# xuhao1/TaichiSLAM

Measured on AMD Instinct MI355X. Metric: depth-frames/s integrated (640x480->512^3 TSDF), higher is better.
Workload: dtype f16 storage / f32 + int64 fixed-point arithmetic; 1 GPU; BASELINE configs[1]: single 640x480 u16 depth stream (sphere room r=3 m, 1 deg/frame) -> DenseTSDF 512^3 / 2 cm, recast_step 2, max_ray 5 m; one stream+submap per GPU

## Files before the change

taichislam_amd/csrc/tsl_common.hpp:

```cpp
#pragma once
#include <cstring>
#include <string.h>
#include <hip/hip_runtime.h>
#include <stdint.h>
#include <string>
#include <vector>
#include "../../include/taichislam_hip.h"

#define TSL_BRK   16
#define TSL_BRK3  4096
#define TSL_EMPTY  (-1)
#define TSL_LOCKED (-2)
#define TSL_FULL   (-3)

namespace tsl {

void set_error(const std::string& s);
#define TSL_HIP(expr) do { hipError_t _e = (expr); if (_e != hipSuccess) { \
    tsl::set_error(std::string(#expr) + ": " + hipGetErrorString(_e)); return TSL_ERR_HIP; } } while (0)
#define TSL_REQUIRE(cond, msg) do { if (!(cond)) { tsl::set_error(msg); return TSL_ERR_ARG; } } while (0)

typedef uint16_t h16;
__device__ __forceinline__ h16 f2h(float x) { _Float16 v = (_Float16)x; return __builtin_bit_cast(h16, v); }
__device__ __forceinline__ float h2f(h16 b) { return (float)__builtin_bit_cast(_Float16, b); }
__device__ __forceinline__ h16 hadd(h16 a, h16 b) { return f2h(h2f(a) + h2f(b)); }
__device__ __forceinline__ h16 hsub(h16 a, h16 b) { return f2h(h2f(a) - h2f(b)); }
__device__ __forceinline__ h16 hmul(h16 a, h16 b) { return f2h(h2f(a) * h2f(b)); }
__device__ __forceinline__ h16 hdiv(h16 a, h16 b) { return f2h(h2f(a) / h2f(b)); }
__device__ __forceinline__ float sqrt_rn(float x) { return sqrtf(x); }
__device__ __forceinline__ float sqrt_rn_norm(float x)
{
    const float y = __builtin_amdgcn_sqrtf(x);
    const float yd = __uint_as_float(__float_as_uint(y) - 1u), yu = __uint_as_float(__float_as_uint(y) + 1u);
    const float ed = __builtin_fmaf(-yd, y, x), eu = __builtin_fmaf(-yu, y, x);
    float r = (ed <= 0.0f) ? yd : y;
    r = (eu > 0.0f) ? yu : r;
    return r;
}
__device__ __forceinline__ h16 hsqrt(h16 a) { return f2h(sqrt_rn(h2f(a))); }

__device__ __forceinline__ float rnd_f(float x)
{
    float r = truncf(x);
    float d = fabsf(x - r);
    if (d >= 0.5f) r += copysignf(1.0f, x);
    return r;
}
__device__ __forceinline__ int rnd_i(float x) { return (int)(x + copysignf(0.49999997f, x)); }
__device__ __forceinline__ int rnd_i_ref(float x) { return (int)rnd_f(x); }
__device__ __forceinline__ int sgn_f(float v) { return (0.0f < v) - (v < 0.0f); }

__device__ __forceinline__ float div_vs(float x, float vs, float rvs, int fast)
{
    if (fast) { const float q0 = x * rvs; const float r = __builtin_fmaf(-q0, vs, x); return __builtin_fmaf(r, rvs, q0); }
    return x / vs;
}

#define TSL_FIX_SCALE 16777216.0f
#define TSL_FIX_INV   (1.0 / 16777216.0)
#define TSL_W_CLAMP   65536.0f
#define TSL_WMAX      1000.0f
__device__ __forceinline__ long long to_fix(float v)
{
    const float q = rintf(v * TSL_FIX_SCALE);
    if (fabsf(q) < 2147483648.0f) return (long long)(int)q;
    return __float2ll_rn(q);
}
__device__ __forceinline__ long long to_fix_wave(float v)
{
    const float q = rintf(v * TSL_FIX_SCALE);
    if (__builtin_expect(__any(!(fabsf(q) < 2147483648.0f)), 0)) return __float2ll_rn(q);
    return (long long)(int)q;
}
__device__ __forceinline__ float from_fix(long long q) { return (float)((double)q * TSL_FIX_INV); }

__device__ __forceinline__ int lane_id() { return __builtin_amdgcn_mbcnt_hi(~0u, __builtin_amdgcn_mbcnt_lo(~0u, 0u)); }
__device__ __forceinline__ int popc64(unsigned long long m) { return __popcll(m); }
__device__ __forceinline__ int rank_below(unsigned long long m)
{ return __builtin_amdgcn_mbcnt_hi((unsigned)(m >> 32), __builtin_amdgcn_mbcnt_lo((unsigned)m, 0u)); }

__device__ __forceinline__ void atomic_add_i64(int64_t* ctr, long long v)
{ __hip_atomic_fetch_add(reinterpret_cast<long long*>(ctr), v, __ATOMIC_RELAXED, __HIP_MEMORY_SCOPE_AGENT); }
__device__ __forceinline__ void wave_count_add(int64_t* ctr, bool pred)
{
    unsigned long long m = __ballot(pred);
    if (m && lane_id() == (int)__builtin_ctzll(m)) atomic_add_i64(ctr, (long long)popc64(m));
}
__device__ __forceinline__ void block_count_add(int64_t* ctr, bool pred)
{
    __shared__ int s_cnt;
    if (threadIdx.x == 0) s_cnt = 0;
    __syncthreads();
    unsigned long long m = __ballot(pred);
    if (m && lane_id() == (int)__builtin_ctzll(m)) atomicAdd(&s_cnt, popc64(m));
    __syncthreads();
    if (threadIdx.x == 0 && s_cnt) atomic_add_i64(ctr, (long long)s_cnt);
    __syncthreads();
}
__device__ __forceinline__ long long wave_sum_ll(long long v)
{
    for (int d = 32; d > 0; d >>= 1) v += __shfl_xor(v, d);
    return v;
}
__device__ __forceinline__ int wave_reserve(int* ctr, bool pred)
{
    unsigned long long m = __ballot(pred);
    if (!m) return -1;
    int leader = (int)__builtin_ctzll(m);
    int base = 0;
    if (lane_id() == leader) base = __hip_atomic_fetch_add(ctr, popc64(m), __ATOMIC_RELAXED, __HIP_MEMORY_SCOPE_AGENT);
    base = __shfl(base, leader);
    return pred ? base + rank_below(m) : -1;
}

__device__ __forceinline__ int block_reserve_n(int* ctr, int n)
{
    __shared__ int s_w[4];
    __shared__ int s_b;
    const int lane = lane_id(), wid = threadIdx.x >> 6;
    int inc = n;
    for (int d = 1; d < 64; d <<= 1) { const int o = __shfl_up(inc, d); if (lane >= d) inc += o; }
    if (lane == 63) s_w[wid] = inc;
    __syncthreads();
    if (threadIdx.x == 0) {
        const int tot = s_w[0] + s_w[1] + s_w[2] + s_w[3];
        s_b = tot ? __hip_atomic_fetch_add(ctr, tot, __ATOMIC_RELAXED, __HIP_MEMORY_SCOPE_AGENT) : 0;
    }
    __syncthreads();
    int off = s_b + inc - n;
    for (int w = 0; w < wid; ++w) off += s_w[w];
    __syncthreads();
    return off;
}

__device__ __forceinline__ int block_reserve(int* ctr, bool pred)
{
    __shared__ int s_w[4];
    __shared__ int s_b;
    const unsigned long long m = __ballot(pred);
    const int wid = threadIdx.x >> 6;
    if (lane_id() == 0) s_w[wid] = popc64(m);
    __syncthreads();
    if (threadIdx.x == 0) {
        const int tot = s_w[0] + s_w[1] + s_w[2] + s_w[3];
        s_b = tot ? __hip_atomic_fetch_add(ctr, tot, __ATOMIC_RELAXED, __HIP_MEMORY_SCOPE_AGENT) : 0;
    }
    __syncthreads();
    int off = s_b + rank_below(m);
    for (int w = 0; w < wid; ++w) off += s_w[w];
    __syncthreads();
    return pred ? off : -1;
}

__device__ __forceinline__ int claim_index_1(int* entry, int* counter, int cap)
{
    int v = __hip_atomic_load(entry, __ATOMIC_RELAXED, __HIP_MEMORY_SCOPE_AGENT);
    while (v == TSL_EMPTY || v == TSL_LOCKED) {
        if (v == TSL_EMPTY) {
            int old = atomicCAS(entry, TSL_EMPTY, TSL_LOCKED);
            if (old == TSL_EMPTY) {
                int idx = __hip_atomic_load(counter, __ATOMIC_RELAXED, __HIP_MEMORY_SCOPE_AGENT);
                if (idx < cap) idx = __hip_atomic_fetch_add(counter, 1, __ATOMIC_RELAXED, __HIP_MEMORY_SCOPE_AGENT);
                __hip_atomic_store(entry, idx >= cap ? TSL_EMPTY : idx, __ATOMIC_RELAXED, __HIP_MEMORY_SCOPE_AGENT);
                return idx >= cap ? TSL_FULL : idx;
            }
            v = old;
        } else {
            __builtin_amdgcn_s_sleep(2);
            v = __hip_atomic_load(entry, __ATOMIC_RELAXED, __HIP_MEMORY_SCOPE_AGENT);
        }
    }
    return v;
}
__device__ __forceinline__ int claim_index(int* entry, int* counter, int cap)
{
    int v = __hip_atomic_load(entry, __ATOMIC_RELAXED, __HIP_MEMORY_SCOPE_AGENT);
    unsigned long long todo = __ballot(v == TSL_EMPTY || v == TSL_LOCKED);
    while (todo) {
        const int leader = (int)__builtin_ctzll(todo);
        const unsigned long long lead = __shfl((unsigned long long)entry, leader);
        int r = 0;
        if (lane_id() == leader) r = claim_index_1(entry, counter, cap);
        r = __shfl(r, leader);
        const bool mine = ((unsigned long long)entry == lead);
        if (mine) v = r;
        todo &= ~__ballot(mine);
    }
    return v;
}

struct MapDev {
    int N, Nz, nbx, nbz, nb3, nsub;
    int hN, hNz;
    int max_bricks;
    int* table;
    uint32_t* tw;
    int8_t* obs;
    int8_t* occ;
    uint16_t* col;
    int* owner;
    uint8_t* touch;
    int* pool_top;
    int* err;
};

__device__ __forceinline__ bool in_volume(const MapDev& M, int i, int j, int k)
{
    return i >= -M.hN && i < M.N - M.hN && j >= -M.hN && j < M.N - M.hN && k >= -M.hNz && k < M.Nz - M.hNz;
}
__device__ __forceinline__ int brick_of(const MapDev& M, int i, int j, int k, int* local)
{
    int ui = i + M.hN, uj = j + M.hN, uk = k + M.hNz;
    *local = ((ui & 15) << 8) | ((uj & 15) << 4) | (uk & 15);
    return ((ui >> 4) * M.nbx + (uj >> 4)) * M.nbz + (uk >> 4);
}
__device__ __forceinline__ int pool_lookup(const MapDev& M, int s, int b)
{ return __hip_atomic_load(M.table + (size_t)s * M.nb3 + b, __ATOMIC_RELAXED, __HIP_MEMORY_SCOPE_AGENT); }
__device__ __forceinline__ int pool_lookup_ro(const MapDev& M, int s, int b) { return M.table[(size_t)s * M.nb3 + b]; }
template <bool COOP = true>
__device__ __forceinline__ int pool_claim(const MapDev& M, int s, int b)
{
    int* e = M.table + (size_t)s * M.nb3 + b;
    int v = __hip_atomic_load(e, __ATOMIC_RELAXED, __HIP_MEMORY_SCOPE_AGENT);
    if (v >= 0) return v;
    v = COOP ? claim_index(e, M.pool_top, M.max_bricks) : claim_index_1(e, M.pool_top, M.max_bricks);
    if (v >= 0) M.owner[v] = s * M.nb3 + b;
    else atomicOr(M.err, 1);
    return v;
}

__device__ __forceinline__ void fuse_write_voxel(const MapDev& G, size_t v, long long qn, long long qd, int c)
{
    const int occ_sum = (int)(int16_t)(c & 0xffff);
    const float num = from_fix(qn), den = from_fix(qd);
    G.tw[v] = (uint32_t)f2h(num / den) | ((uint32_t)f2h(den) << 16);
    G.obs[v] = 1;
    G.occ[v] = (int8_t)occ_sum;
}


}
```

taichislam_amd/csrc/tsl_integrate.hip:

```cpp
#include "tsl_tsdf.hpp"
#include <hip/hip_ext.h>

namespace tsl {

#ifdef TSL_TIMING
#define TSL_T0() const int _wv = (blockIdx.x * (int)blockDim.x + (int)threadIdx.x) >> 6
#define TSL_TICK(F, k) do { long long _n = wall_clock64(); if (lane_id() == 0 && _wv < 16384) (F).dbg[_wv * 16 + (k)] = _n; } while (0)
#else
#define TSL_T0() do {} while (0)
#define TSL_TICK(F, k) do {} while (0)
#endif

#define SCATTER_TILE 4096

struct RayRegs { float pf0, pf1, pf2, d0, d1, d2, P0, P1, P2, w; long long qden; int n; };

__device__ __forceinline__ uint32_t wave_min_u32(uint32_t v)
{
    for (int d = 32; d > 0; d >>= 1) { const uint32_t o = (uint32_t)__shfl_xor((int)v, d); v = o < v ? o : v; }
    return v;
}
__device__ __forceinline__ RayRegs make_ray(const uint4 rec, int n, const FrameParams& P)
{
    RayRegs R;
    R.n = n;
    R.pf0 = h2f((h16)(rec.x & 0xffffu)); R.pf1 = h2f((h16)(rec.x >> 16)); R.pf2 = h2f((h16)(rec.y & 0xffffu));
    R.d0 = h2f((h16)(rec.y >> 16)); R.d1 = h2f((h16)(rec.z & 0xffffu)); R.d2 = h2f((h16)(rec.z >> 16));
    R.w = __uint_as_float(rec.w);
    R.qden = to_fix(R.w);
    R.P0 = R.pf0 + P.T[0]; R.P1 = R.pf1 + P.T[1]; R.P2 = R.pf2 + P.T[2];
    return R;
}
template <bool WITH_N = true>
__device__ __forceinline__ RayRegs load_ray(const FrameDev& F, const FrameParams& P, int r) { return make_ray(F.rayA[r], WITH_N ? F.rayN[r] : 0, P); }
__device__ __forceinline__ void step_voxel(const RayRegs& R, const FrameParams& P, int j, float* x, int* xi)
{
    const float jf = (float)j;
    x[0] = (R.d0 * jf) * P.vs + P.T[0]; x[1] = (R.d1 * jf) * P.vs + P.T[1]; x[2] = (R.d2 * jf) * P.vs + P.T[2];
    xi[0] = rnd_i(div_vs(x[0], P.vs, P.rvs, P.fastdiv)); xi[1] = rnd_i(div_vs(x[1], P.vs, P.rvs, P.fastdiv)); xi[2] = rnd_i(div_vs(x[2], P.vs, P.rvs, P.fastdiv));
}
__device__ __forceinline__ long long step_term(const RayRegs& R, const float* x)
{
    const float v0 = R.P0 - x[0], v1 = R.P1 - x[1], v2 = R.P2 - x[2];
    const float s2 = (v0 * v0 + v1 * v1) + v2 * v2;
    const float dist = s2 >= 1.2621774483536189e-29f ? sqrt_rn_norm(s2) : sqrt_rn(s2);
    const float dot = (v0 * R.pf0 + v1 * R.pf1) + v2 * R.pf2;
    const float sd = dist * (float)sgn_f(dot);
    return to_fix_wave(R.w * sd);
}
template <bool COOP = true>
__device__ __forceinline__ void mark_occupied(const MapDev& M, const FrameParams& P, const RayRegs& R)
{
    const int oi = rnd_i(div_vs(R.P0, P.vs, P.rvs, P.fastdiv)), oj = rnd_i(div_vs(R.P1, P.vs, P.rvs, P.fastdiv)), ok = rnd_i(div_vs(R.P2, P.vs, P.rvs, P.fastdiv));
    if (in_volume(M, oi, oj, ok)) {
        int l; const int b = brick_of(M, oi, oj, ok, &l);
        const int p = pool_claim<COOP>(M, P.slot, b);
        if (p >= 0) M.occ[(size_t)p * TSL_BRK3 + l] = 1;
    }
}
template <bool COOP = true>
__device__ __forceinline__ int frame_slot_slow(const MapDev& M, const FrameDev& F, int s, int b)
{
    const int sl = COOP ? claim_index(F.slot_tab + b, &F.counters[1], F.max_frame_bricks) : claim_index_1(F.slot_tab + b, &F.counters[1], F.max_frame_bricks);
    if (sl >= 0) {
        const int p = pool_claim<COOP>(M, s, b);
        if (p >= 0) { F.touched[sl] = p; F.touched_b[sl] = b; }
        else return -1;
    } else frame_fail(M, F, 2);
    return sl;
}
__device__ __forceinline__ int frame_slot(const MapDev& M, const FrameDev& F, int s, int b)
{
    const int sl = F.slot_tab[b];
    return sl >= 0 ? sl : frame_slot_slow(M, F, s, b);
}

__device__ __forceinline__ uint32_t apply_update(uint32_t old, long long qnum, long long qden)
{
    const float num = from_fix(qnum), den = from_fix(qden);
    const h16 T0 = (h16)(old & 0xffffu), W0 = (h16)(old >> 16);
    const h16 Tn = f2h((h2f(hmul(T0, W0)) + num) / (h2f(W0) + den));
    float wn = h2f(W0) + den; if (TSL_WMAX < wn) wn = TSL_WMAX;
    return (uint32_t)Tn | ((uint32_t)f2h(wn) << 16);
}
__device__ __forceinline__ uint32_t apply_update_f(uint32_t old, float num, float den)
{
    const h16 T0 = (h16)(old & 0xffffu), W0 = (h16)(old >> 16);
    const h16 Tn = f2h((h2f(hmul(T0, W0)) + num) / (h2f(W0) + den));
    float wn = h2f(W0) + den; if (TSL_WMAX < wn) wn = TSL_WMAX;
    return (uint32_t)Tn | ((uint32_t)f2h(wn) << 16);
}

template <int VARIANT>
__global__ void __launch_bounds__(256) k_integrate(MapDev M, FrameDev F, const FrameParams* __restrict__ Pp)
{
    const FrameParams& P = *Pp;
    const int split = P.split;
    const int gid = blockIdx.x * 256 + threadIdx.x;
    const int r = gid / split, sub = gid - r * split;
    const int nrays = *F.nrays;
    const bool live = r < nrays;
    long long n_ok = 0, n_oob = 0;
    RayRegs R; R.n = 0; R.qden = 0;
    if (live) { R = load_ray(F, P, r); if (sub == 0) mark_occupied(M, P, R); }
    int cur_b = -1; unsigned long long* cur_acc = nullptr;
    int nmax = R.n;
    if (VARIANT == 1) { for (int d = 32; d > 0; d >>= 1) { int o = __shfl_xor(nmax, d); nmax = o > nmax ? o : nmax; } }
    const int iters = (nmax + split - 1) / split;
    for (int it = 0; it < iters; ++it) {
        const int j = 1 + sub + it * split;
        const bool act = live && j <= R.n;
        unsigned long long* dst = nullptr;
        long long qn = 0;
        if (act) {
            float x[3]; int xi[3];
            step_voxel(R, P, j, x, xi);
            if (in_volume(M, xi[0], xi[1], xi[2])) {
                qn = step_term(R, x);
                int l; const int b = brick_of(M, xi[0], xi[1], xi[2], &l);
                if (b != cur_b) { cur_b = b; const int sl = frame_slot(M, F, P.slot, b); cur_acc = sl >= 0 ? F.acc + (size_t)sl * (TSL_BRK3 * 2) : nullptr; }
                if (cur_acc) { dst = cur_acc + (size_t)l * 2; ++n_ok; }
            } else ++n_oob;
        }
        if (VARIANT == 1) {
            const unsigned long long m = __ballot(dst != nullptr);
            if (m) {
                const int leader = (int)__builtin_ctzll(m);
                const unsigned long long lead = __shfl((unsigned long long)dst, leader);
                const bool same = (dst == nullptr) || ((unsigned long long)dst == lead);
                if (__all(same)) {
                    const long long sn = wave_sum_ll(dst ? qn : 0), sdn = wave_sum_ll(dst ? R.qden : 0);
                    if (lane_id() == leader) {
                        __hip_atomic_fetch_add(dst, (unsigned long long)sn, __ATOMIC_RELAXED, __HIP_MEMORY_SCOPE_AGENT);
                        __hip_atomic_fetch_add(dst + 1, (unsigned long long)sdn, __ATOMIC_RELAXED, __HIP_MEMORY_SCOPE_AGENT);
                    }
                    continue;
                }
            }
        }
        if (dst) {
            __hip_atomic_fetch_add(dst, (unsigned long long)qn, __ATOMIC_RELAXED, __HIP_MEMORY_SCOPE_AGENT);
            __hip_atomic_fetch_add(dst + 1, (unsigned long long)R.qden, __ATOMIC_RELAXED, __HIP_MEMORY_SCOPE_AGENT);
        }
    }
    n_ok = wave_sum_ll(n_ok); n_oob = wave_sum_ll(n_oob);
    if (lane_id() == 0) {
        if (n_ok) atomic_add_i64(&F.stats->steps, n_ok);
        if (n_oob) atomic_add_i64(&F.stats->steps_oob, n_oob);
    }
}

__global__ void __launch_bounds__(256) k_finalize(MapDev M, FrameDev F, const int* list, const int* nlist)
{
    const int ntouched = min(F.counters[1], F.max_frame_bricks);
    const int nwork = list ? min(*nlist, F.max_frame_bricks) : ntouched;
    long long uniq = 0;
    for (int q = blockIdx.x; q < nwork; q += gridDim.x) {
        const int sl = list ? list[q] : q;
        const int p = F.touched[sl];
        if (threadIdx.x == 0) M.touch[p] = 1;
        ulonglong2* acc = reinterpret_cast<ulonglong2*>(F.acc + (size_t)sl * (TSL_BRK3 * 2));
        uint32_t* tw = M.tw + (size_t)p * TSL_BRK3;
        int8_t* obs = M.obs + (size_t)p * TSL_BRK3;
        ulonglong2 a[TSL_BRK3 / 256]; uint32_t old[TSL_BRK3 / 256];
#pragma unroll
        for (int q = 0; q < TSL_BRK3 / 256; ++q) { a[q] = acc[q * 256 + threadIdx.x]; old[q] = tw[q * 256 + threadIdx.x]; }
#pragma unroll
        for (int q = 0; q < TSL_BRK3 / 256; ++q) {
            const int l = q * 256 + threadIdx.x;
            if (a[q].y != 0ull) {
                tw[l] = apply_update(old[q], (long long)a[q].x, (long long)a[q].y);
                obs[l] = 1;
                acc[l] = make_ulonglong2(0ull, 0ull);
                ++uniq;
            }
        }
    }
    for (int sl = blockIdx.x * 256 + threadIdx.x; sl < ntouched; sl += gridDim.x * 256) F.slot_tab[F.touched_b[sl]] = TSL_EMPTY;
    uniq = wave_sum_ll(uniq);
    if (lane_id() == 0 && uniq) atomic_add_i64(&F.stats->unique, uniq);
    if (!list && blockIdx.x == 0 && threadIdx.x == 0) F.stats->bricks = ntouched;
}

__device__ __forceinline__ int axis_coord(float d, float T, const FrameParams& P, int j) { return rnd_i(div_vs((d * (float)j) * P.vs + T, P.vs, P.rvs, P.fastdiv)); }
__device__ __forceinline__ int axis_cell(int c, int h, int N, int nb) { const int u = c + h; return u < 0 ? -1 : (u >= N ? nb : (u >> 4)); }

__device__ __forceinline__ int next_axis_event(float d, float inv_d, float T, const FrameParams& P, float t_over_vs, int j, int jb, int cell, int h, int N, int nb)
{
    if (j >= jb) return jb + 1;
    int bound;
    bool up;
    if (d > 0.0f) { if (cell >= nb) return jb + 1; up = true; bound = (cell < 0 ? 0 : min((cell + 1) * 16, N)) - h; }
    else if (d < 0.0f) { if (cell < 0) return jb + 1; up = false; bound = (cell >= nb ? N - 1 : cell * 16 - 1) - h; }
    else return jb + 1;
    const float est = ((float)bound + (up ? -0.5f : 0.5f) - t_over_vs) * inv_d;
    int e = (int)fminf(fmaxf(ceilf(est), (float)(j + 1)), (float)jb);
    #define TSL_PRED(q) (up ? (axis_coord(d, T, P, (q)) >= bound) : (axis_coord(d, T, P, (q)) <= bound))
    if (TSL_PRED(e)) { while (e - 1 > j && TSL_PRED(e - 1)) --e; }
    else { ++e; while (e <= jb && !TSL_PRED(e)) ++e; }
    #undef TSL_PRED
    return e;
}

#define LH_SIZE 1024
#define LH_EMPTY (-1)
template <int LOG2 = 10>
__device__ __forceinline__ int lh_slot(int* keys, int b)
{
    unsigned h = ((unsigned)b * 2654435761u) >> (32 - LOG2);
    for (int probe = 0; probe < (1 << LOG2); ++probe) {
        const int k = keys[h];
        if (k == b) return (int)h;
        if (k == LH_EMPTY) { const int old = atomicCAS(&keys[h], LH_EMPTY, b); if (old == LH_EMPTY || old == b) return (int)h; }
        h = (h + 1) & ((1u << LOG2) - 1u);
    }
    return -1;
}

#define SEG_RAY_SLOTS 16
#define SEG_LH_LOG2 9
#define SEG_LH (1 << SEG_LH_LOG2)
template <bool FUSED>
__global__ void __launch_bounds__(256) k_segments(MapDev M, BatchDev B)
{
    if ((int)blockIdx.y >= B.n) return;
    const FrameDev& F = B.f[blockIdx.y];
    const FrameParams& P = *B.p[blockIdx.y];
    __shared__ int s_key[SEG_LH];
    __shared__ int s_cnt[SEG_LH];
    TSL_T0();
    TSL_TICK(F, 8);
    for (int i = threadIdx.x; i < SEG_LH; i += 256) { s_key[i] = LH_EMPTY; s_cnt[i] = 0; }
    __syncthreads();
    TSL_TICK(F, 0);

    const int split = P.split;
    const int gid = blockIdx.x * 256 + threadIdx.x;
    const int r = gid / split, sub = gid - r * split;
    const int nrays = FUSED ? F.counters[6] : *F.nrays;
    long long n_ok = 0, n_oob = 0;
    const bool working = __any(r < nrays);
    const int spl = SEG_RAY_SLOTS / split;
    unsigned long long* myseg = F.seg + (size_t)gid * spl;
    int nslot = 0;
    bool ok = r < nrays;
    uint4 rec = make_uint4(0, 0, 0, 0);
    int nsteps = 0;
    if (FUSED) {
        const int lane = threadIdx.x & 63;
        bool big = false;
        int gn = 0, sl = 0;
        uint32_t first = 0;
        unsigned long long vkey = 0ull;
        ok = false;
        if (r < nrays && sub == 0) {
            sl = F.act[r];
            const uint4* sp = reinterpret_cast<const uint4*>(F.htab + sl);
            const uint4 w0 = sp[0], w1 = sp[1], w2 = sp[2], w3 = sp[3];
            vkey = ((unsigned long long)w0.x | ((unsigned long long)w0.y << 32)) - 1ull;
            gn = (int)w0.z;
            if (gn > H_INL) big = true;
            else {
                uint32_t id[H_INL] = { w0.w, w1.x, w1.y, w1.z, w1.w, w2.x, w2.y, w2.z, w2.w, w3.x, w3.y, w3.z, w3.w };
                uint2 pl[H_INL];
#pragma unroll
                for (int q = 0; q < H_INL; ++q) {
                    if (q >= gn) id[q] = 0xffffffffu;
                    pl[q] = q < gn ? F.pix[id[q]] : make_uint2(0u, 0u);
                }
                PixAcc A = {};
                for (int k = 0; k < gn; ++k) {
                    uint32_t best = 0xffffffffu; uint2 bp = make_uint2(0u, 0u);
#pragma unroll
                    for (int q = 0; q < H_INL; ++q) { const bool t = id[q] < best; best = t ? id[q] : best; bp.x = t ? pl[q].x : bp.x; bp.y = t ? pl[q].y : bp.y; }
#pragma unroll
                    for (int q = 0; q < H_INL; ++q) id[q] = id[q] == best ? 0xffffffffu : id[q];
                    if (k == 0) first = best;
                    if (P.tex) acc_colour(P, F, best, A);
                    acc_payload(bp, A);
                }
                ok = finish_ray(P, F, A, first, &rec, &nsteps);
            }
        }
        for (unsigned long long bm = __ballot(big); bm; bm &= bm - 1ull) {
            const int src = (int)__builtin_ctzll(bm);
            const int n = __shfl(gn, src), sl0 = __shfl(sl, src);
            const unsigned long long vk = ((unsigned long long)(uint32_t)__shfl((int)(vkey >> 32), src) << 32) | (unsigned long long)(uint32_t)__shfl((int)(uint32_t)vkey, src);
            const int nblk = (n + H_INL - 1) / H_INL;
            const uint32_t hmask = (1u << P.hlog2) - 1u;
            auto find_block = [&](int bq) -> int {
                if (bq == 0) return sl0;
                const unsigned long long k2 = h_key(vk, bq);
                uint32_t h = h_hash64(k2, P.hlog2);
                for (uint32_t probe = 0; probe <= hmask; ++probe) {
                    const unsigned long long cur = F.htab[h].key;
                    if (cur == k2) return (int)h;
                    if (cur == H_EMPTY) return -1;
                    h = (h + 1u) & hmask;
                }
                return -1;
            };
            const int mine = lane < nblk ? find_block(lane) : -1;
            const bool too_many = n > GROUP_BIG_CAP;
            if (too_many && lane == 0) atomicOr(M.err, 8);
            PixAcc A = {};
            long long last = -1; uint32_t f0 = 0;
            for (int k = 0; k < n && !too_many; ++k) {
                uint32_t best = 0xffffffffu;
                for (int bq = lane; bq < nblk; bq += 64) {
                    const int hs = bq == lane ? mine : find_block(bq);
                    if (hs < 0) continue;
                    const int cb = min(H_INL, n - bq * H_INL);
                    const uint32_t* ids = F.htab[hs].pix;
                    for (int q = 0; q < cb; ++q) { const uint32_t v = ids[q]; if ((long long)v > last && v < best) best = v; }
                }
                best = wave_min_u32(best);
                if (best == 0xffffffffu) break;
                if (k == 0) f0 = best;
                acc_pixel(P, F, best, A);
                last = (long long)best;
            }
            uint4 rc; int ns = 0;
            const bool k2 = A.cnt == n && finish_ray(P, F, A, f0, &rc, &ns, lane == src);
            if (lane == src) { rec = rc; nsteps = ns; ok = k2; first = f0; }
        }
        if (r < nrays && sub == 0) {
            F.rayA[r] = rec; F.rayFirst[r] = first;
            if (P.seq) {
                uint32_t u[3];
#pragma unroll
                for (int a = 0; a < 3; ++a) {
                    unsigned long long x = (vkey >> (2 - a)) & 0x1249249249249249ull;
                    x = (x | (x >> 2)) & 0x10c30c30c30c30c3ull; x = (x | (x >> 4)) & 0x100f00f00f00f00full; x = (x | (x >> 8)) & 0x1f0000ff0000ffull;
                    x = (x | (x >> 16)) & 0x1f00000000ffffull; x = (x | (x >> 32)) & 0x1fffffull;
                    u[a] = (uint32_t)x;
                }
                const unsigned long long nblk = (unsigned long long)(P.pcl_ext / P.pcl_blk), blk = (unsigned long long)P.pcl_blk;
                const unsigned long long kb = ((u[0] / P.pcl_blk) * nblk + (u[1] / P.pcl_blk)) * nblk + (u[2] / P.pcl_blk);
                const unsigned long long kl = ((u[0] % P.pcl_blk) * blk + (u[1] % P.pcl_blk)) * blk + (u[2] % P.pcl_blk);
                reinterpret_cast<unsigned long long*>(F.keys)[r] = kb * blk * blk * blk + kl;
                F.rayN[r] = ok ? nsteps : 0;
            }
        }
        block_count_add(&F.stats->v_pcl, r < nrays && sub == 0);
        block_count_add(&F.stats->v_skipped, r < nrays && sub == 0 && !ok);
        if (gid == 0) *F.nrays = nrays;
        const int src = lane - sub;
        rec.x = (uint32_t)__shfl((int)rec.x, src); rec.y = (uint32_t)__shfl((int)rec.y, src); rec.z = (uint32_t)__shfl((int)rec.z, src); rec.w = (uint32_t)__shfl((int)rec.w, src);
        nsteps = __shfl(nsteps, src);
        ok = __shfl((int)ok, src) != 0;
    }
    if (ok) {
        const RayRegs R = FUSED ? make_ray(rec, nsteps, P) : load_ray(F, P, r);
        if (sub == 0) mark_occupied(M, P, R);
        TSL_TICK(F, 1);
        const int len = (R.n + split - 1) / split;
        const int ja = 1 + sub * len, jb = min(R.n, ja + len - 1);
        const float d[3] = { R.d0, R.d1, R.d2 };
        const float id[3] = { __builtin_amdgcn_rcpf(R.d0), __builtin_amdgcn_rcpf(R.d1), __builtin_amdgcn_rcpf(R.d2) };
        const float tv[3] = { P.T[0] / P.vs, P.T[1] / P.vs, P.T[2] / P.vs };
        const int hh[3] = { M.hN, M.hN, M.hNz }, NN[3] = { M.N, M.N, M.Nz }, nb[3] = { M.nbx, M.nbx, M.nbz };
        if (ja <= jb) {
            int cell[3], ev[3];
#pragma unroll
            for (int a = 0; a < 3; ++a) {
                cell[a] = axis_cell(axis_coord(d[a], P.T[a], P, ja), hh[a], NN[a], nb[a]);
                ev[a] = next_axis_event(d[a], id[a], P.T[a], P, tv[a], ja, jb, cell[a], hh[a], NN[a], nb[a]);
            }
            int j = ja;
            while (j <= jb) {
                const int e = min(min(ev[0], ev[1]), ev[2]);
                const bool inside = cell[0] >= 0 && cell[0] < nb[0] && cell[1] >= 0 && cell[1] < nb[1] && cell[2] >= 0 && cell[2] < nb[2];
                if (inside) {
                    const int b = (cell[0] * M.nbx + cell[1]) * M.nbz + cell[2];
                    n_ok += e - j;
                    for (int j0 = j; j0 < e; j0 += SEG_MAX_CNT) {
                        const int cnt = min(e - j0, SEG_MAX_CNT);
                        const unsigned long long en = ((unsigned long long)b << STG_B_SHIFT) | ((unsigned long long)r << (SEG_CNT_BITS + SEG_J_BITS)) |
                                                      ((unsigned long long)j0 << SEG_CNT_BITS) | (unsigned long long)cnt;
                        bool stored = true;
                        if (nslot < spl) myseg[nslot++] = en;
                        else {
                            const long long pos = (long long)nrays * SEG_RAY_SLOTS + __hip_atomic_fetch_add(&F.counters[2], 1, __ATOMIC_RELAXED, __HIP_MEMORY_SCOPE_AGENT);
                            if (pos < F.seg_cap) F.seg[pos] = en; else { stored = false; frame_fail(M, F, 4); }
                        }
                        if (stored) {
                            const int hs = lh_slot<SEG_LH_LOG2>(s_key, b);
                            if (hs >= 0) atomicAdd(&s_cnt[hs], 1);
                            else if (__hip_atomic_fetch_add(&F.bhist[b], 1, __ATOMIC_RELAXED, __HIP_MEMORY_SCOPE_AGENT) == 0) {
                                const int q = __hip_atomic_fetch_add(&F.counters[1], 1, __ATOMIC_RELAXED, __HIP_MEMORY_SCOPE_AGENT);
                                if (q < F.max_frame_bricks) F.act_b[q] = b; else frame_fail(M, F, 2);
                            }
                        }
                    }
                } else n_oob += e - j;
                j = e;
                if (j > jb) break;
#pragma unroll
                for (int a = 0; a < 3; ++a) if (ev[a] == j) {
                    cell[a] += d[a] > 0.0f ? 1 : -1;
                    ev[a] = next_axis_event(d[a], id[a], P.T[a], P, tv[a], j, jb, cell[a], hh[a], NN[a], nb[a]);
                }
            }
        }
    }
    if (r < nrays) for (int q = nslot; q < spl; ++q) myseg[q] = ~0ull;
    TSL_TICK(F, 2);
    __syncthreads();
    TSL_TICK(F, 3);
    TSL_TICK(F, 5);
    for (int i = threadIdx.x; i < SEG_LH; i += 256) {
        const int c = s_cnt[i];
        const int b = c ? s_key[i] : 0;
        const bool first = c && __hip_atomic_fetch_add(&F.bhist[b], c, __ATOMIC_RELAXED, __HIP_MEMORY_SCOPE_AGENT) == 0;
        const int q = wave_reserve(&F.counters[1], first);
        if (first) { if (q < F.max_frame_bricks) F.act_b[q] = b; else frame_fail(M, F, 2); }
    }
    TSL_TICK(F, 6);
#ifdef TSL_TIMING
    if (lane_id() == 0 && _wv < 16384) F.dbg[_wv * 16 + 15] = working;
#endif
    (void)working;
    n_ok = wave_sum_ll(n_ok); n_oob = wave_sum_ll(n_oob);
    {
        __shared__ long long s_steps[2];
        if (threadIdx.x == 0) { s_steps[0] = 0; s_steps[1] = 0; }
        __syncthreads();
        if (lane_id() == 0) {
            if (n_ok) atomicAdd(reinterpret_cast<unsigned long long*>(&s_steps[0]), (unsigned long long)n_ok);
            if (n_oob) atomicAdd(reinterpret_cast<unsigned long long*>(&s_steps[1]), (unsigned long long)n_oob);
        }
        __syncthreads();
        if (threadIdx.x == 0) {
            if (s_steps[0]) atomic_add_i64(&F.stats->steps, s_steps[0]);
            if (s_steps[1]) atomic_add_i64(&F.stats->steps_oob, s_steps[1]);
        }
    }
}

__device__ __forceinline__ int plan_class(int w) { return w >= 2560 ? 0 : (w >= 1280 ? 1 : (w >= 512 ? 2 : 3)); }
__global__ void __launch_bounds__(256) k_plan(MapDev M, BatchDev B, int psegs, int unit_max, int unit_half)
{
    if ((int)blockIdx.y >= B.n) return;
    const int y = blockIdx.y;
    const FrameDev& F = B.f[y];
    const int listed = F.counters[1];
    const int nact = min(listed, F.max_frame_bricks);
    if ((int)blockIdx.x * 256 >= nact && blockIdx.x) return;
    const int i = blockIdx.x * 256 + threadIdx.x;
    int v = 0, b = 0, np = 0, pcls = -1, ucls = -1, tm = 0, wb = 0, tmu = 0, tmp = 0, wu = 0;
    if (i < nact) {
        b = F.act_b[i];
        v = F.bhist[b];
        int vq[TSL_NB];
#pragma unroll
        for (int q = 0; q < TSL_NB; ++q) { vq[q] = q < B.n ? B.f[q].bhist[b] : 0; if (vq[q] > 0) tm |= 1 << q; wb += vq[q]; }
        if (wb > unit_max) { tmp = tm; }
        else if (wb > unit_half) {
            int acc = 0;
#pragma unroll
            for (int q = 0; q < TSL_NB; ++q) if ((tm >> q) & 1) { if (2 * acc < wb) { tmu |= 1 << q; wu += vq[q]; } else tmp |= 1 << q; acc += vq[q]; }
        } else { tmu = tm; wu = wb; }
        if (tmu && (tmu & -tmu) == (1 << y)) ucls = plan_class(wu);
        if (((tmp >> y) & 1) && v > 0) { np = (v + psegs - 1) / psegs; pcls = plan_class((v + np - 1) / np); }
    }
    const int off = block_reserve_n(&F.counters[3], v);
    const int s0 = block_reserve_n(&B.f[0].counters[HDR_SLAB], np);
    int p0 = 0, u0 = 0;
    for (int c = 0; c < PLAN_NCLS; ++c) {
        const int q = block_reserve_n(&F.counters[HDR_PARTS + c], pcls == c ? np : 0); if (pcls == c) p0 = q;
        const int u = block_reserve_n(&B.f[0].counters[HDR_UNITS + c], ucls == c ? 1 : 0); if (ucls == c) u0 = u;
    }
    if (i < nact) {
        F.boffset[b] = off;
        F.bnseg[b] = v;
        const int pool = (np || ucls >= 0) ? pool_claim<false>(M, B.p[y]->slot, b) : -1;
        if (ucls >= 0) {
            if (u0 < B.f[0].unit_cap) B.f[0].unit_tab[(size_t)ucls * B.f[0].unit_cap + u0] = make_int4(b, wu, pool, tmu);
            else for (int q = 0; q < B.n; ++q) if ((tm >> q) & 1) frame_fail(M, B.f[q], 2);
        }
        if (np && pool >= 0) {
            if ((tmp & -tmp) == (1 << y)) {
                const int hi = __hip_atomic_fetch_add(&B.f[0].counters[HDR_HEAVY], 1, __ATOMIC_RELAXED, __HIP_MEMORY_SCOPE_AGENT);
                if (hi < B.f[0].max_frame_bricks) B.f[0].heavy_tab[hi] = make_int4(b, pool, tmp, 0);
                else for (int q = 0; q < B.n; ++q) if ((tm >> q) & 1) frame_fail(M, B.f[q], 2);
            }
            if (s0 + np > F.max_frame_bricks || np >= (1 << PART_NP_BITS) || p0 + np > F.part_cap) frame_fail(M, F, 2);
            else {
                F.bslab[b] = s0 | (np << SLAB_SLOT_BITS);
                const int per = (v + np - 1) / np;
                int4* tab = F.part_tab + (size_t)pcls * F.part_cap;
                for (int k = 0; k < np; ++k) {
                    const int pos = k * per, n = min(v, pos + per) - pos;
                    tab[p0 + k] = make_int4(off + pos, (int)((uint32_t)n | ((uint32_t)np << 16)), pool, s0 + k);
                }
            }
        }
    }
    if (i == 0) { F.stats->bricks = listed; if (listed > F.max_frame_bricks) frame_fail(M, F, 2); }
}

__global__ void __launch_bounds__(256) k_scatter(BatchDev B)
{
    if ((int)blockIdx.y >= B.n) return;
    const FrameDev& F = B.f[blockIdx.y];
    __shared__ int s_key[LH_SIZE];
    __shared__ int s_cnt[LH_SIZE];
    __shared__ int s_base[LH_SIZE];
    if (B.p[blockIdx.y]->group) {
        const int na = F.counters[6], nx = F.counters[7];
        for (int i = blockIdx.x * 256 + threadIdx.x; i < na + nx; i += gridDim.x * 256) {
            HSlot* const hs = F.htab + (i < na ? F.act[i] : F.actx[i - na]);
            hs->key = H_EMPTY; hs->cnt = 0;
        }
    }
    const int total = (int)min((long long)*F.nrays * SEG_RAY_SLOTS + F.counters[2], (long long)F.seg_cap);
    const int ntiles = (total + SCATTER_TILE - 1) / SCATTER_TILE;
    for (int tile = blockIdx.x; tile < ntiles; tile += gridDim.x) {
        for (int i = threadIdx.x; i < LH_SIZE; i += 256) { s_key[i] = LH_EMPTY; s_cnt[i] = 0; }
        __syncthreads();
        const int t0 = tile * SCATTER_TILE;
        unsigned long long key[SCATTER_TILE / 256]; int rank[SCATTER_TILE / 256]; int hs[SCATTER_TILE / 256];
#pragma unroll
        for (int q = 0; q < SCATTER_TILE / 256; ++q) {
            const int i = t0 + q * 256 + threadIdx.x;
            rank[q] = -1; hs[q] = -1;
            if (i < total) {
                key[q] = F.seg[i];
                if (key[q] != ~0ull) {
                    const int b = (int)(key[q] >> STG_B_SHIFT);
                    hs[q] = lh_slot<10>(s_key, b);
                    if (hs[q] >= 0) rank[q] = atomicAdd(&s_cnt[hs[q]], 1);
                    else rank[q] = F.boffset[b] + __hip_atomic_fetch_add(&F.bcursor[b], 1, __ATOMIC_RELAXED, __HIP_MEMORY_SCOPE_AGENT);
                }
            }
        }
        __syncthreads();
        for (int i = threadIdx.x; i < LH_SIZE; i += 256) {
            const int c = s_cnt[i];
            if (c) { const int b = s_key[i]; s_base[i] = F.boffset[b] + __hip_atomic_fetch_add(&F.bcursor[b], c, __ATOMIC_RELAXED, __HIP_MEMORY_SCOPE_AGENT); }
        }
        __syncthreads();
#pragma unroll
        for (int q = 0; q < SCATTER_TILE / 256; ++q)
            if (rank[q] >= 0) F.seg_sorted[(hs[q] >= 0 ? s_base[hs[q]] : 0) + rank[q]] = key[q];
        __syncthreads();
    }
}

#ifdef TSL_NOSWZ
__device__ __forceinline__ int acc_swz5(int l) { return l; }
#else
__device__ __forceinline__ int acc_swz5(int l) { return l ^ (((l >> 8) ^ (l >> 5)) & 31); }
#endif
struct StepK { float vs, rvs, T0, T1, T2; int hN, hNz; };

template <bool FASTDIV>
__device__ __forceinline__ void step_eval(const RayRegs& R, const StepK& K, int j, int* slot, float* qf)
{
    const float jf = (float)j;
    const float x0 = (R.d0 * jf) * K.vs + K.T0, x1 = (R.d1 * jf) * K.vs + K.T1, x2 = (R.d2 * jf) * K.vs + K.T2;
    const int i0 = rnd_i(div_vs(x0, K.vs, K.rvs, FASTDIV ? 1 : 0)), i1 = rnd_i(div_vs(x1, K.vs, K.rvs, FASTDIV ? 1 : 0)), i2 = rnd_i(div_vs(x2, K.vs, K.rvs, FASTDIV ? 1 : 0));
    *slot = acc_swz5((((i0 + K.hN) & 15) << 8) | (((i1 + K.hN) & 15) << 4) | ((i2 + K.hNz) & 15));
    const float v0 = R.P0 - x0, v1 = R.P1 - x1, v2 = R.P2 - x2;
    const float s2 = (v0 * v0 + v1 * v1) + v2 * v2;
    const float dist = sqrt_rn_norm(fmaxf(s2, 1.2621774483536189e-29f));
    const float dot = (v0 * R.pf0 + v1 * R.pf1) + v2 * R.pf2;
    const float sd = dot == 0.0f ? 0.0f : copysignf(dist, dot);
    *qf = rintf((R.w * sd) * TSL_FIX_SCALE);
}

__device__ __forceinline__ bool fits_i32(long long q) { return q == (long long)(int)q; }
__device__ __forceinline__ float from_fix32(long long q) { return (float)(int)q * (float)TSL_FIX_INV; }

#define FLUSH_CHUNK 4
template <int N>
__device__ __forceinline__ void apply_chunk(const uint32_t* old, const long long* qn, const long long* qd, uint32_t* nv, bool all_small)
{
    if (all_small) {
#pragma unroll
        for (int q = 0; q < N; ++q) nv[q] = apply_update_f(old[q], from_fix32(qn[q]), from_fix32(qd[q]));
    } else {
#pragma unroll
        for (int q = 0; q < N; ++q) nv[q] = apply_update_f(old[q], from_fix(qn[q]), from_fix(qd[q]));
    }
}

__device__ __forceinline__ int uni(int v) { return __builtin_amdgcn_readfirstlane(v); }
#define IT_UNIT 0
#define IT_POOL 1
#define IT_SLAB 2
#define IT_NP   3
#define IT_TMALL 4
#define IT_FMASK 5
#define IT_OFF  6
#define IT_N    (IT_OFF + TSL_NB)
#define IT_WORDS (IT_N + TSL_NB + 2)
#define NRANGE (PLAN_NCLS * (TSL_NB + 1))

template <bool TEX, bool FASTDIV, int NT, int SPT, int WPE>
__global__ void __launch_bounds__(NT, WPE) k_integrate_batch(MapDev M, BatchDev B, int kind)
{
    constexpr int CSEGS = SPT * NT, VPT = TSL_BRK3 / NT, CH = VPT < FLUSH_CHUNK ? VPT : FLUSH_CHUNK;
    static_assert(VPT <= 16, "the written / first-touch masks hold 16 voxels per thread");
#ifdef TSL_EXP_SLOT16
    __shared__ ulonglong2 s_acc[TSL_BRK3];
#define S_NUM(i) s_acc[i].x
#define S_DEN(i) s_acc[i].y
#else
    __shared__ unsigned long long s_num[TSL_BRK3];
    __shared__ unsigned long long s_den[TSL_BRK3];
#define S_NUM(i) s_num[i]
#define S_DEN(i) s_den[i]
#endif
    __shared__ unsigned long long s_keys[CSEGS];
    __shared__ uint32_t s_win[TEX ? TSL_BRK3 : 1];
    __shared__ int s_bin[64];
    __shared__ int s_claim[2];
    __shared__ int s_uq[TSL_NB];
    __shared__ int s_cum[NRANGE + 1];
    __shared__ int s_it[3][IT_WORDS];
    uint32_t okmask = 0u;
#pragma unroll
    for (int q = 0; q < TSL_NB; ++q) if (q < B.n) {
        const FrameDev& Fq = B.f[q];
        if (Fq.counters[HDR_FAIL] == 0) okmask |= 1u << q;
        const int nact = min(Fq.counters[1], Fq.max_frame_bricks);
        for (int i = blockIdx.x * NT + threadIdx.x; i < nact; i += gridDim.x * NT) { const int b = Fq.act_b[i]; Fq.bhist[b] = 0; Fq.bcursor[b] = 0; }
    }
    if (threadIdx.x < TSL_NB) s_uq[threadIdx.x] = 0;
    if (threadIdx.x == 0) {
        int acc = 0, k = 0;
#ifdef TSL_CLASS_MAJOR
        for (int c = 0; c < PLAN_NCLS; ++c) {
            s_cum[k++] = acc; acc += min(B.f[0].counters[HDR_UNITS + c], B.f[0].unit_cap);
            for (int q = 0; q < TSL_NB; ++q) { s_cum[k++] = acc; if ((okmask >> q) & 1u) acc += min(B.f[q].counters[HDR_PARTS + c], B.f[q].part_cap); }
        }
#else
        for (int c = 0; c < PLAN_NCLS; ++c) { s_cum[k++] = acc; if (kind != 2) acc += min(B.f[0].counters[HDR_UNITS + c], B.f[0].unit_cap); }
        for (int c = 0; c < PLAN_NCLS; ++c)
            for (int q = 0; q < TSL_NB; ++q) { s_cum[k++] = acc; if (kind != 1 && ((okmask >> q) & 1u)) acc += min(B.f[q].counters[HDR_PARTS + c], B.f[q].part_cap); }
#endif
        s_cum[NRANGE] = acc;
        s_claim[0] = __hip_atomic_fetch_add(&B.f[0].counters[kind == 2 ? HDR_CLAIM2 : HDR_CLAIM], 1, __ATOMIC_RELAXED, __HIP_MEMORY_SCOPE_AGENT);
    }
    __syncthreads();
    const int total = uni(s_cum[NRANGE]);
    int* const claim = &B.f[0].counters[kind == 2 ? HDR_CLAIM2 : HDR_CLAIM];
    auto entry_of = [&](int r, int* kq) -> int4 {
        int k = 0;
#pragma unroll
        for (int j = 1; j < NRANGE; ++j) k += r >= uni(s_cum[j]) ? 1 : 0;
#ifdef TSL_CLASS_MAJOR
        const int local = r - uni(s_cum[k]), cls = k / (TSL_NB + 1), sub = k - cls * (TSL_NB + 1);
#else
        const int local = r - uni(s_cum[k]), cls = k < PLAN_NCLS ? k : (k - PLAN_NCLS) / TSL_NB, sub = k < PLAN_NCLS ? 0 : 1 + (k - PLAN_NCLS) % TSL_NB;
#endif
        *kq = sub - 1;
        if (sub == 0) return B.f[0].unit_tab[(size_t)cls * B.f[0].unit_cap + local];
        const FrameDev& Fq = B.f[sub - 1];
        return Fq.part_tab[(size_t)cls * Fq.part_cap + local];
    };
    auto info_of = [&](const int4 e, int kq, int* io, int* in) {
        *io = 0; *in = 0;
        const int q = threadIdx.x;
        if (q < TSL_NB) {
            if (kq < 0) { if ((((uint32_t)e.w) & okmask) >> q & 1u) { *io = B.f[q].boffset[e.x]; *in = B.f[q].bnseg[e.x]; } }
            else if (q == kq) { *io = e.x; *in = e.y & 0xffff; }
        }
    };
    auto commit = [&](int slot, const int4 e, int kq, int io, int in) {
        int* it = s_it[slot];
        if (threadIdx.x < TSL_NB) { it[IT_OFF + threadIdx.x] = io; it[IT_N + threadIdx.x] = in; }
        if (threadIdx.x == 0) {
            const uint32_t tm = kq < 0 ? (uint32_t)e.w & okmask : 1u << kq;
            uint32_t fm = tm;
            int pool = e.z;
            if (fm == 0u) { fm = 1u; pool = -1; }
            it[IT_UNIT] = kq < 0 ? 1 : 0; it[IT_POOL] = pool; it[IT_SLAB] = kq < 0 ? 0 : e.w; it[IT_NP] = kq < 0 ? 1 : (e.y >> 16) & ((1 << PART_NP_BITS) - 1);
            it[IT_TMALL] = (int)tm; it[IT_FMASK] = (int)fm;
        }
    };
    const int r0 = uni(s_claim[0]);
    if (r0 >= total) return;
    { int kq, io, in; const int4 e = entry_of(r0, &kq); info_of(e, kq, &io, &in); commit(0, e, kq, io, in); }
    __syncthreads();
    auto steps_of = [&](int sl, uint32_t fm) -> int {
        int n = 0;
#pragma unroll
        for (int q = 0; q < TSL_NB; ++q) if ((fm >> q) & 1u) n += max(1, (uni(s_it[sl][IT_N + q]) + CSEGS - 1) / CSEGS);
        return n;
    };
    long long uniq = 0;
    int t = 0, slot = 0, c = 0; (void)t;
    int n_known = 0;
    bool exhausted = false;
    int f = __builtin_ctz((uint32_t)uni(s_it[0][IT_FMASK]));

    unsigned long long kk[SPT]; uint4 recs[SPT]; uint32_t wids[SPT];
#define TSL_SORT_DEAL(KIN, NSEG, FD)                                                                                    \
    {                                                                                                                   \
        int rr[SPT];                                                                                                    \
        _Pragma("unroll") for (int q = 0; q < SPT; ++q) {                                                               \
            const int i = q * NT + (int)threadIdx.x; rr[q] = -1;                                                        \
            if (i < (NSEG)) rr[q] = atomicAdd(&s_bin[63 - (int)(KIN[q] & 63ull)], 1);                                   \
        }                                                                                                               \
        __syncthreads();                                                                                                \
// ... 405 lines not shown
```

Measured before the change: 34350 frames/s.

## Factor ray brick traversal into shared helper and early-exit idle segment blocks

Moves the per-axis brick-boundary event walk into a host/device header as a lambda-driven traversal. The new loop picks one axis per step through scalar selects, so next_axis_event is inlined once instead of three times; this aims to shrink code size and register pressure. It also returns early from blocks whose rays are all beyond nrays, which skips their shared hash-table init and the later flush. The selection chains add a few ALU ops per event, and the early return reads the ray count before the barrier.

```diff
diff --git a/taichislam_amd/csrc/tsl_common.hpp b/taichislam_amd/csrc/tsl_common.hpp
--- a/taichislam_amd/csrc/tsl_common.hpp
+++ b/taichislam_amd/csrc/tsl_common.hpp
@@ -6,6 +6,7 @@
 #include <string>
 #include <vector>
 #include "../../include/taichislam_hip.h"
+#include "tsl_segments.hpp"
 
 #define TSL_BRK   16
 #define TSL_BRK3  4096
@@ -46,15 +47,8 @@
     if (d >= 0.5f) r += copysignf(1.0f, x);
     return r;
 }
-__device__ __forceinline__ int rnd_i(float x) { return (int)(x + copysignf(0.49999997f, x)); }
 __device__ __forceinline__ int rnd_i_ref(float x) { return (int)rnd_f(x); }
 __device__ __forceinline__ int sgn_f(float v) { return (0.0f < v) - (v < 0.0f); }
-
-__device__ __forceinline__ float div_vs(float x, float vs, float rvs, int fast)
-{
-    if (fast) { const float q0 = x * rvs; const float r = __builtin_fmaf(-q0, vs, x); return __builtin_fmaf(r, rvs, q0); }
-    return x / vs;
-}
 
 #define TSL_FIX_SCALE 16777216.0f
 #define TSL_FIX_INV   (1.0 / 16777216.0)
diff --git a/taichislam_amd/csrc/tsl_integrate.hip b/taichislam_amd/csrc/tsl_integrate.hip
--- a/taichislam_amd/csrc/tsl_integrate.hip
+++ b/taichislam_amd/csrc/tsl_integrate.hip
@@ -182,25 +182,6 @@
     if (!list && blockIdx.x == 0 && threadIdx.x == 0) F.stats->bricks = ntouched;
 }
 
-__device__ __forceinline__ int axis_coord(float d, float T, const FrameParams& P, int j) { return rnd_i(div_vs((d * (float)j) * P.vs + T, P.vs, P.rvs, P.fastdiv)); }
-__device__ __forceinline__ int axis_cell(int c, int h, int N, int nb) { const int u = c + h; return u < 0 ? -1 : (u >= N ? nb : (u >> 4)); }
-
-__device__ __forceinline__ int next_axis_event(float d, float inv_d, float T, const FrameParams& P, float t_over_vs, int j, int jb, int cell, int h, int N, int nb)
-{
-    if (j >= jb) return jb + 1;
-    int bound;
-    bool up;
-    if (d > 0.0f) { if (cell >= nb) return jb + 1; up = true; bound = (cell < 0 ? 0 : min((cell + 1) * 16, N)) - h; }
-    else if (d < 0.0f) { if (cell < 0) return jb + 1; up = false; bound = (cell >= nb ? N - 1 : cell * 16 - 1) - h; }
-    else return jb + 1;
-    const float est = ((float)bound + (up ? -0.5f : 0.5f) - t_over_vs) * inv_d;
-    int e = (int)fminf(fmaxf(ceilf(est), (float)(j + 1)), (float)jb);
-    #define TSL_PRED(q) (up ? (axis_coord(d, T, P, (q)) >= bound) : (axis_coord(d, T, P, (q)) <= bound))
-    if (TSL_PRED(e)) { while (e - 1 > j && TSL_PRED(e - 1)) --e; }
-    else { ++e; while (e <= jb && !TSL_PRED(e)) ++e; }
-    #undef TSL_PRED
-    return e;
-}
 
 #define LH_SIZE 1024
 #define LH_EMPTY (-1)
@@ -230,14 +211,15 @@
     __shared__ int s_cnt[SEG_LH];
     TSL_T0();
     TSL_TICK(F, 8);
+    const int split = P.split;
+    const int nrays = FUSED ? F.counters[6] : *F.nrays;
+    if (blockIdx.x != 0 && (int)(blockIdx.x * 256u / (unsigned)split) >= nrays) return;
     for (int i = threadIdx.x; i < SEG_LH; i += 256) { s_key[i] = LH_EMPTY; s_cnt[i] = 0; }
     __syncthreads();
     TSL_TICK(F, 0);
 
-    const int split = P.split;
     const int gid = blockIdx.x * 256 + threadIdx.x;
     const int r = gid / split, sub = gid - r * split;
-    const int nrays = FUSED ? F.counters[6] : *F.nrays;
     long long n_ok = 0, n_oob = 0;
     const bool working = __any(r < nrays);
     const int spl = SEG_RAY_SLOTS / split;
@@ -356,53 +338,36 @@
         TSL_TICK(F, 1);
         const int len = (R.n + split - 1) / split;
         const int ja = 1 + sub * len, jb = min(R.n, ja + len - 1);
-        const float d[3] = { R.d0, R.d1, R.d2 };
-        const float id[3] = { __builtin_amdgcn_rcpf(R.d0), __builtin_amdgcn_rcpf(R.d1), __builtin_amdgcn_rcpf(R.d2) };
-        const float tv[3] = { P.T[0] / P.vs, P.T[1] / P.vs, P.T[2] / P.vs };
-        const int hh[3] = { M.hN, M.hN, M.hNz }, NN[3] = { M.N, M.N, M.Nz }, nb[3] = { M.nbx, M.nbx, M.nbz };
-        if (ja <= jb) {
-            int cell[3], ev[3];
-#pragma unroll
-            for (int a = 0; a < 3; ++a) {
-                cell[a] = axis_cell(axis_coord(d[a], P.T[a], P, ja), hh[a], NN[a], nb[a]);
-                ev[a] = next_axis_event(d[a], id[a], P.T[a], P, tv[a], ja, jb, cell[a], hh[a], NN[a], nb[a]);
-            }
-            int j = ja;
-            while (j <= jb) {
-                const int e = min(min(ev[0], ev[1]), ev[2]);
-                const bool inside = cell[0] >= 0 && cell[0] < nb[0] && cell[1] >= 0 && cell[1] < nb[1] && cell[2] >= 0 && cell[2] < nb[2];
-                if (inside) {
-                    const int b = (cell[0] * M.nbx + cell[1]) * M.nbz + cell[2];
-                    n_ok += e - j;
-                    for (int j0 = j; j0 < e; j0 += SEG_MAX_CNT) {
-                        const int cnt = min(e - j0, SEG_MAX_CNT);
-                        const unsigned long long en = ((unsigned long long)b << STG_B_SHIFT) | ((unsigned long long)r << (SEG_CNT_BITS + SEG_J_BITS)) |
-                                                      ((unsigned long long)j0 << SEG_CNT_BITS) | (unsigned long long)cnt;
-                        bool stored = true;
-                        if (nslot < spl) myseg[nslot++] = en;
-                        else {
-                            const long long pos = (long long)nrays * SEG_RAY_SLOTS + __hip_atomic_fetch_add(&F.counters[2], 1, __ATOMIC_RELAXED, __HIP_MEMORY_SCOPE_AGENT);
-                            if (pos < F.seg_cap) F.seg[pos] = en; else { stored = false; frame_fail(M, F, 4); }
-                        }
-                        if (stored) {
-                            const int hs = lh_slot<SEG_LH_LOG2>(s_key, b);
-                            if (hs >= 0) atomicAdd(&s_cnt[hs], 1);
-                            else if (__hip_atomic_fetch_add(&F.bhist[b], 1, __ATOMIC_RELAXED, __HIP_MEMORY_SCOPE_AGENT) == 0) {
-                                const int q = __hip_atomic_fetch_add(&F.counters[1], 1, __ATOMIC_RELAXED, __HIP_MEMORY_SCOPE_AGENT);
-                                if (q < F.max_frame_bricks) F.act_b[q] = b; else frame_fail(M, F, 2);
-                            }
+        SegGeom G;
+        G.vs = P.vs; G.rvs = P.rvs; G.fastdiv = P.fastdiv;
+        G.T[0] = P.T[0]; G.T[1] = P.T[1]; G.T[2] = P.T[2];
+        G.h[0] = M.hN; G.h[1] = M.hN; G.h[2] = M.hNz; G.N[0] = M.N; G.N[1] = M.N; G.N[2] = M.Nz; G.nb[0] = M.nbx; G.nb[1] = M.nbx; G.nb[2] = M.nbz;
+        ray_brick_runs(G, R.d0, R.d1, R.d2, ja, jb, [&](int j, int e, const int (&cell)[3]) {
+            const bool inside = cell[0] >= 0 && cell[0] < M.nbx && cell[1] >= 0 && cell[1] < M.nbx && cell[2] >= 0 && cell[2] < M.nbz;
+            if (inside) {
+                const int b = (cell[0] * M.nbx + cell[1]) * M.nbz + cell[2];
+                n_ok += e - j;
+                for (int j0 = j; j0 < e; j0 += SEG_MAX_CNT) {
+                    const int cnt = min(e - j0, SEG_MAX_CNT);
+                    const unsigned long long en = ((unsigned long long)b << STG_B_SHIFT) | ((unsigned long long)r << (SEG_CNT_BITS + SEG_J_BITS)) |
+                                                  ((unsigned long long)j0 << SEG_CNT_BITS) | (unsigned long long)cnt;
+                    bool stored = true;
+                    if (nslot < spl) myseg[nslot++] = en;
+                    else {
+                        const long long pos = (long long)nrays * SEG_RAY_SLOTS + __hip_atomic_fetch_add(&F.counters[2], 1, __ATOMIC_RELAXED, __HIP_MEMORY_SCOPE_AGENT);
+                        if (pos < F.seg_cap) F.seg[pos] = en; else { stored = false; frame_fail(M, F, 4); }
+                    }
+                    if (stored) {
+                        const int hs = lh_slot<SEG_LH_LOG2>(s_key, b);
+                        if (hs >= 0) atomicAdd(&s_cnt[hs], 1);
+                        else if (__hip_atomic_fetch_add(&F.bhist[b], 1, __ATOMIC_RELAXED, __HIP_MEMORY_SCOPE_AGENT) == 0) {
+                            const int q = __hip_atomic_fetch_add(&F.counters[1], 1, __ATOMIC_RELAXED, __HIP_MEMORY_SCOPE_AGENT);
+                            if (q < F.max_frame_bricks) F.act_b[q] = b; else frame_fail(M, F, 2);
                         }
                     }
-                } else n_oob += e - j;
-                j = e;
-                if (j > jb) break;
-#pragma unroll
-                for (int a = 0; a < 3; ++a) if (ev[a] == j) {
-                    cell[a] += d[a] > 0.0f ? 1 : -1;
-                    ev[a] = next_axis_event(d[a], id[a], P.T[a], P, tv[a], j, jb, cell[a], hh[a], NN[a], nb[a]);
-                }
-            }
-        }
+                }
+            } else n_oob += e - j;
+        });
     }
     if (r < nrays) for (int q = nslot; q < spl; ++q) myseg[q] = ~0ull;
     TSL_TICK(F, 2);
diff --git a/taichislam_amd/csrc/tsl_segments.hpp b/taichislam_amd/csrc/tsl_segments.hpp
--- /dev/null
+++ b/taichislam_amd/csrc/tsl_segments.hpp
@@ -0,0 +1,83 @@
+#pragma once
+#include <math.h>
+
+#if defined(__HIP__) || defined(__CUDACC__)
+#define TSL_HD __host__ __device__ __forceinline__
+#else
+#define TSL_HD inline
+#endif
+
+namespace tsl {
+
+TSL_HD int rnd_i(float x) { return (int)(x + __builtin_copysignf(0.49999997f, x)); }
+
+TSL_HD float div_vs(float x, float vs, float rvs, int fast)
+{
+    if (fast) { const float q0 = x * rvs; const float r = __builtin_fmaf(-q0, vs, x); return __builtin_fmaf(r, rvs, q0); }
+    return x / vs;
+}
+
+struct SegGeom { float vs, rvs; int fastdiv; float T[3]; int h[3], N[3], nb[3]; };
+
+TSL_HD float seg_rcp(float d)
+{
+#if defined(__HIP_DEVICE_COMPILE__)
+    return __builtin_amdgcn_rcpf(d);
+#else
+    return 1.0f / d;
+#endif
+}
+
+TSL_HD int axis_coord(float d, float T, const SegGeom& G, int j) { return rnd_i(div_vs((d * (float)j) * G.vs + T, G.vs, G.rvs, G.fastdiv)); }
+TSL_HD int axis_cell(int c, int h, int N, int nb) { const int u = c + h; return u < 0 ? -1 : (u >= N ? nb : (u >> 4)); }
+
+TSL_HD int next_axis_event(float d, float inv_d, float T, const SegGeom& G, float t_over_vs, int j, int jb, int cell, int h, int N, int nb)
+{
+    if (j >= jb) return jb + 1;
+    int bound;
+    bool up;
+    if (d > 0.0f) { if (cell >= nb) return jb + 1; up = true; bound = (cell < 0 ? 0 : (cell + 1) * 16 < N ? (cell + 1) * 16 : N) - h; }
+    else if (d < 0.0f) { if (cell < 0) return jb + 1; up = false; bound = (cell >= nb ? N - 1 : cell * 16 - 1) - h; }
+    else return jb + 1;
+    const float est = ((float)bound + (up ? -0.5f : 0.5f) - t_over_vs) * inv_d;
+    int e = (int)__builtin_fminf(__builtin_fmaxf(__builtin_ceilf(est), (float)(j + 1)), (float)jb);
+    #define TSL_PRED(q) (up ? (axis_coord(d, T, G, (q)) >= bound) : (axis_coord(d, T, G, (q)) <= bound))
+    if (TSL_PRED(e)) { while (e - 1 > j && TSL_PRED(e - 1)) --e; }
+    else { ++e; while (e <= jb && !TSL_PRED(e)) ++e; }
+    #undef TSL_PRED
+    return e;
+}
+
+template <class Emit>
+TSL_HD void ray_brick_runs(const SegGeom& G, float d0, float d1, float d2, int ja, int jb, Emit&& emit)
+{
+    if (ja > jb) return;
+    const float i0 = seg_rcp(d0), i1 = seg_rcp(d1), i2 = seg_rcp(d2);
+    const float t0 = G.T[0] / G.vs, t1 = G.T[1] / G.vs, t2 = G.T[2] / G.vs;
+    int c0 = axis_cell(axis_coord(d0, G.T[0], G, ja), G.h[0], G.N[0], G.nb[0]) - (d0 > 0.0f ? 1 : -1);
+    int c1 = axis_cell(axis_coord(d1, G.T[1], G, ja), G.h[1], G.N[1], G.nb[1]) - (d1 > 0.0f ? 1 : -1);
+    int c2 = axis_cell(axis_coord(d2, G.T[2], G, ja), G.h[2], G.N[2], G.nb[2]) - (d2 > 0.0f ? 1 : -1);
+    int e0 = ja, e1 = ja, e2 = ja;
+    int j = ja;
+    for (;;) {
+        for (;;) {
+            const int a = e0 == j ? 0 : (e1 == j ? 1 : (e2 == j ? 2 : 3));
+            if (a == 3) break;
+            const float da = a == 0 ? d0 : (a == 1 ? d1 : d2);
+            const int ca = (a == 0 ? c0 : (a == 1 ? c1 : c2)) + (da > 0.0f ? 1 : -1);
+            const int ea = next_axis_event(da, a == 0 ? i0 : (a == 1 ? i1 : i2), a == 0 ? G.T[0] : (a == 1 ? G.T[1] : G.T[2]), G,
+                                           a == 0 ? t0 : (a == 1 ? t1 : t2), j, jb, ca,
+                                           a == 0 ? G.h[0] : (a == 1 ? G.h[1] : G.h[2]), a == 0 ? G.N[0] : (a == 1 ? G.N[1] : G.N[2]),
+                                           a == 0 ? G.nb[0] : (a == 1 ? G.nb[1] : G.nb[2]));
+            c0 = a == 0 ? ca : c0; c1 = a == 1 ? ca : c1; c2 = a == 2 ? ca : c2;
+            e0 = a == 0 ? ea : e0; e1 = a == 1 ? ea : e1; e2 = a == 2 ? ea : e2;
+        }
+        const int e = e0 < e1 ? (e0 < e2 ? e0 : e2) : (e1 < e2 ? e1 : e2);
+        const int cell[3] = { c0, c1, c2 };
+        emit(j, e, cell);
+        j = e;
+        if (j > jb) break;
+    }
+}
+
+}
```

New measurement: 33440 frames/s. -2.6%, worse.
